# alexj94/future_urban_scene_generation

Hardware: AMD Instinct MI355X
Metric: synthesised vehicle crops/sec @256x256 (higher is better)
Workload: dtype f32 tensors; conv contraction as 3 fp16 MFMA products of scaled (hi, lo) operand splits, f32 accumulate (error vs fp64 <= 1.3x the exact-f32 MFMA kernel's: observed 0.96-1.27x over 12 operand scales x 5 layers; range-guarded; exact-f32 leg in precision_legs)

## Files before the change

future_urban_scene_generation_amd/csrc/conv_bneck.hip:

```cpp
#include "conv_kernel_h3.h"

namespace fusg {

struct BneckK {
    const float* x; const float* res; float* dst;
    long xsn, xsh, xsw, rsn, rsh, rsw, dsn, dsh, dsw;
    const float* pre_scale; const float* pre_shift;
    const _Float16* w1; const _Float16* w2; const _Float16* w3;
    const float* b1; const float* b2; const float* b3;
    const float* s1; const float* s2; const float* s3;
    const float* zeros;
    int* status;
    int B, H, W, Cin, tiles_x, tiles_y;
    int touch_w;
};

constexpr int BN_HP = 100;
constexpr int BN_SROWS = 112;
constexpr size_t bneck_lds(int planes) { return (size_t)(2 * BN_SROWS * 32 + 2 * (planes / 32) * BN_HP * 32) * sizeof(_Float16); }

template <int CT> struct WFrag { h8 f[CT][2]; };

#ifdef FUSG_BNECK_STAMPS
__device__ unsigned long long g_bneck_stamps[64 * 12];
#define FUSG_STAMP(i) do { if (threadIdx.x == 0 && blockIdx.x < 64) g_bneck_stamps[blockIdx.x * 12 + (i)] = __builtin_amdgcn_s_memtime(); } while (0)
#define FUSG_STAMP_RT(i) do { if (threadIdx.x == 0 && blockIdx.x < 64) g_bneck_stamps[blockIdx.x * 12 + (i)] = __builtin_amdgcn_s_memrealtime(); } while (0)
#else
#define FUSG_STAMP(i) do {} while (0)
#define FUSG_STAMP_RT(i) do {} while (0)
#endif

__device__ __forceinline__ f32x4 mfma16(const h8 a, const h8 b, const f32x4 c) {
    return __builtin_amdgcn_mfma_f32_16x16x32_f16(a, b, c, 0, 0, 0);
}

template <int P>
__global__ __launch_bounds__(256, 2) void hg_bneck_h3(const BneckK k) {
    constexpr int NCH = P / 32;
    constexpr int CT1 = P / 64, CT3 = P / 32;
    extern __shared__ __attribute__((aligned(16))) _Float16 smem_h[];
    _Float16* Sh = smem_h;
    _Float16* Sl = Sh + BN_SROWS * 32;
    _Float16* Th = Sl + BN_SROWS * 32;
    _Float16* Tl = Th + NCH * BN_HP * 32;
    _Float16* Uh = Th;
    _Float16* Ul = Th + NCH * 64 * 32;

    const int t = threadIdx.x, lane = t & 63, wave = t >> 6;
    const int lp = lane & 15, lg = lane >> 4;
    FUSG_STAMP_RT(8);
    FUSG_STAMP(0);
    const int tile = xcd_tile();
    const int tpi = k.tiles_x * k.tiles_y;
    const int b = tile / tpi, t2 = tile - b * tpi;
    const int ty = t2 / k.tiles_x, tx = t2 - ty * k.tiles_x;
    const int oy0 = ty * 8, ox0 = tx * 8;
    float amax = 0.f;
    const float ninf = -__builtin_inff();

    if (k.touch_w && gridDim.x <= TOUCH_MAX_WGS / 2) {
        void* dummy = (char*)smem_h + bneck_lds(P);
        const long n1 = (long)(k.Cin >> 5) * NCH * 4096, n2 = (long)9 * NCH * NCH * 4096, n3 = (long)NCH * 2 * NCH * 4096;
        for (long o = (long)t * 128; o < n1; o += 256 * 128) l2_touch((const char*)k.w1 + o, dummy);
        for (long o = (long)t * 128; o < n2; o += 256 * 128) l2_touch((const char*)k.w2 + o, dummy);
        for (long o = (long)t * 128; o < n3; o += 256 * 128) l2_touch((const char*)k.w3 + o, dummy);
    }

    const int kc = t & 7;
    const float* xp[4];
    int soff[4];
    unsigned sval = 0, sexist = 0;
#pragma unroll
    for (int j = 0; j < 4; ++j) {
        const int item = t + 256 * j, pix = item >> 3;
        xp[j] = k.zeros;
        soff[j] = 0;
        if (item < BN_SROWS * 8) {
            sexist |= 1u << j;
            soff[j] = pix * 32 + ((((kc >> 1) ^ (((pix >> 2) & 1) << 1)) << 3) | ((kc & 1) << 2));
            if (pix < BN_HP) {
                const int hy = pix / 10, hx = pix - hy * 10;
                const int iy = oy0 - 1 + hy, ix = ox0 - 1 + hx;
                if ((unsigned)iy < (unsigned)k.H && (unsigned)ix < (unsigned)k.W) {
                    sval |= 1u << j;
                    xp[j] = k.x + (long)b * k.xsn + (long)iy * k.xsh + (long)ix * k.xsw + kc * 4;
                }
            }
        }
    }
    f32x4 hreg[4], sc = {1.f, 1.f, 1.f, 1.f}, sh = {0.f, 0.f, 0.f, 0.f};
    auto issue = [&](int c) {
        sc = *(const f32x4*)(k.pre_scale + c * 32 + kc * 4);
        sh = *(const f32x4*)(k.pre_shift + c * 32 + kc * 4);
#pragma unroll
        for (int j = 0; j < 4; ++j) hreg[j] = *(const f32x4*)(((sval >> j) & 1u) ? xp[j] + c * 32 : k.zeros);
    };
    auto commit = [&]() {
#pragma unroll
        for (int j = 0; j < 4; ++j) {
            f32x4 v = hreg[j];
            const bool ok = (sval >> j) & 1u;
#pragma unroll
            for (int c = 0; c < 4; ++c) { const float y = fmaf(v[c], sc[c], sh[c]); v[c] = ok ? y : 0.f; }
            h4 hi, lo;
            split4(v, 0.f, hi, lo, amax);
            if ((sexist >> j) & 1u) { *(h4*)(Sh + soff[j]) = hi; *(h4*)(Sl + soff[j]) = lo; }
        }
    };
    auto load_w = [&](auto& F, const _Float16* w, int slab, int nt32, int gct0) {
        constexpr int CT = sizeof(F.f) / sizeof(F.f[0]);
#pragma unroll
        for (int j = 0; j < CT; ++j) {
            const int gct = gct0 + j;
            const _Float16* p = w + ((long)((slab * nt32 + (gct >> 1)) * 2 + (gct & 1)) * 2) * 512 + lane * 8;
            F.f[j][0] = *(const h8*)(p);
            F.f[j][1] = *(const h8*)(p + 512);
        }
    };

    f32x4 acc1[7][CT1];
#pragma unroll
    for (int i = 0; i < 7; ++i)
#pragma unroll
        for (int j = 0; j < CT1; ++j) acc1[i][j] = f32x4{0.f, 0.f, 0.f, 0.f};
    const int sfrag = lp * 32 + ((lg ^ (((lp >> 2) & 1) << 1)) << 3);
    auto compute1 = [&](const WFrag<CT1>& F) {
        h8 bs[CT1];
#pragma unroll
        for (int j = 0; j < CT1; ++j) bs[j] = scale_m11(F.f[j][0]);
#pragma unroll
        for (int i0 = 0; i0 < 7; i0 += 2) {
            const int n = i0 + 1 < 7 ? 2 : 1;
            h8 xh[2], xl[2];
#pragma unroll
            for (int i = 0; i < 2; ++i)
                if (i < n) { xh[i] = *(const h8*)(Sh + (i0 + i) * 512 + sfrag); xl[i] = *(const h8*)(Sl + (i0 + i) * 512 + sfrag); }
#pragma unroll
            for (int term = 0; term < 3; ++term)
#pragma unroll
                for (int i = 0; i < 2; ++i)
                    if (i < n) {
#pragma unroll
                        for (int j = 0; j < CT1; ++j)
                            acc1[i0 + i][j] = mfma16(term == 0 ? F.f[j][0] : term == 1 ? F.f[j][1] : bs[j], term == 2 ? xl[i] : xh[i], acc1[i0 + i][j]);
                    }
        }
    };

    const int nch1 = k.Cin >> 5;
    WFrag<CT1> wA, wB;
    FUSG_STAMP(1);
    issue(0);
    load_w(wA, k.w1, 0, NCH, wave * CT1);
    for (int c = 0; c < nch1; c += 2) {
        commit();
        __syncthreads();
        if (c + 1 < nch1) { issue(c + 1); load_w(wB, k.w1, c + 1, NCH, wave * CT1); }
        compute1(wA);
        __syncthreads();
        if (c + 1 >= nch1) break;
        commit();
        __syncthreads();
        if (c + 2 < nch1) { issue(c + 2); load_w(wA, k.w1, c + 2, NCH, wave * CT1); }
        compute1(wB);
        __syncthreads();
    }

    FUSG_STAMP(2);
    WFrag<CT1> w0, w1, w2;
    load_w(w0, k.w2, 0, NCH, wave * CT1);
    load_w(w1, k.w2, NCH, NCH, wave * CT1);
    const int sub = (lg & 1) << 2;
    {
#pragma unroll
        for (int j = 0; j < CT1; ++j) {
            const int gct = wave * CT1 + j;
            const int n0 = gct * 16 + lg * 4;
            const f32x4 bias = *(const f32x4*)(k.b1 + n0), wsc = *(const f32x4*)(k.s1 + n0);
            const int g = (gct & 1) * 2 + (lg >> 1);
#pragma unroll
            for (int i = 0; i < 7; ++i) {
                const int pix = i * 16 + lp;
                const int hy = pix / 10, hx = pix - hy * 10;
                const int iy = oy0 - 1 + hy, ix = ox0 - 1 + hx;
                const bool ok = pix < BN_HP && (unsigned)iy < (unsigned)k.H && (unsigned)ix < (unsigned)k.W;
                f32x4 v;
#pragma unroll
                for (int r = 0; r < 4; ++r) { const float y = fmaxf(fmaf(acc1[i][j][r], wsc[r], bias[r]), 0.f); v[r] = ok ? y : 0.f; }
                h4 hi, lo;
                split4<false>(v, ninf, hi, lo, amax);
                if (pix < BN_HP) {
                    const int o = ((gct >> 1) * BN_HP + pix) * 32 + ((g ^ ((hy & 1) << 1)) << 3) + sub;
                    *(h4*)(Th + o) = hi;
                    *(h4*)(Tl + o) = lo;
                }
            }
        }
    }
    __syncthreads();
    FUSG_STAMP(3);

    f32x4 acc2[4][CT1];
#pragma unroll
    for (int i = 0; i < 4; ++i)
#pragma unroll
        for (int j = 0; j < CT1; ++j) acc2[i][j] = f32x4{0.f, 0.f, 0.f, 0.f};
    const int prow = lp >> 3, pcol = lp & 7;
    const int tfrag = (prow * 10 + pcol) * 32;
    auto compute2 = [&](const WFrag<CT1>& F, int c, int tap) {
        const int ky = tap / 3, kx = tap - ky * 3;
        const int o = c * (BN_HP * 32) + tfrag + (ky * 10 + kx) * 32 + ((lg ^ (((prow + ky) & 1) << 1)) << 3);
        h8 xh[4], xl[4], bs[CT1];
#pragma unroll
        for (int i = 0; i < 4; ++i) { xh[i] = *(const h8*)(Th + o + i * 640); xl[i] = *(const h8*)(Tl + o + i * 640); }
#pragma unroll
        for (int j = 0; j < CT1; ++j) bs[j] = scale_m11(F.f[j][0]);
#pragma unroll
        for (int term = 0; term < 3; ++term)
#pragma unroll
            for (int i = 0; i < 4; ++i)
#pragma unroll
                for (int j = 0; j < CT1; ++j)
                    acc2[i][j] = mfma16(term == 0 ? F.f[j][0] : term == 1 ? F.f[j][1] : bs[j], term == 2 ? xl[i] : xh[i], acc2[i][j]);
    };
    for (int c = 0; c < NCH; ++c) {
#pragma unroll
        for (int tap = 0; tap < 9; tap += 3) {
            const int s2 = c * 9 + tap + 2;
            auto slab_of = [](int s) { const int cc = s / 9; return (s - cc * 9) * NCH + cc; };
            load_w(w2, k.w2, slab_of(s2), NCH, wave * CT1);
            compute2(w0, c, tap);
            if (s2 + 1 < NCH * 9) load_w(w0, k.w2, slab_of(s2 + 1), NCH, wave * CT1);
            compute2(w1, c, tap + 1);
            if (s2 + 2 < NCH * 9) load_w(w1, k.w2, slab_of(s2 + 2), NCH, wave * CT1);
            compute2(w2, c, tap + 2);
        }
    }
    FUSG_STAMP(4);
    __syncthreads();

    WFrag<CT3> v0, v1;
    load_w(v0, k.w3, 0, 2 * NCH, wave * CT3);
    {
#pragma unroll
        for (int j = 0; j < CT1; ++j) {
            const int gct = wave * CT1 + j;
            const int n0 = gct * 16 + lg * 4;
            const f32x4 bias = *(const f32x4*)(k.b2 + n0), wsc = *(const f32x4*)(k.s2 + n0);
            const int g = (gct & 1) * 2 + (lg >> 1);
#pragma unroll
            for (int i = 0; i < 4; ++i) {
                f32x4 v;
#pragma unroll
                for (int r = 0; r < 4; ++r) v[r] = fmaxf(fmaf(acc2[i][j][r], wsc[r], bias[r]), 0.f);
                h4 hi, lo;
                split4<false>(v, ninf, hi, lo, amax);
                const int o = ((gct >> 1) * 64 + i * 16 + lp) * 32 + ((g ^ (((lp >> 2) & 1) << 1)) << 3) + sub;
                *(h4*)(Uh + o) = hi;
                *(h4*)(Ul + o) = lo;
            }
        }
    }
    __syncthreads();
    FUSG_STAMP(5);

    f32x4 acc3[4][CT3];
#pragma unroll
    for (int i = 0; i < 4; ++i)
#pragma unroll
        for (int j = 0; j < CT3; ++j) acc3[i][j] = f32x4{0.f, 0.f, 0.f, 0.f};
    auto compute3 = [&](const WFrag<CT3>& F, int c) {
        h8 xh[4], xl[4];
#pragma unroll
        for (int i = 0; i < 4; ++i) { xh[i] = *(const h8*)(Uh + c * 2048 + i * 512 + sfrag); xl[i] = *(const h8*)(Ul + c * 2048 + i * 512 + sfrag); }
        h8 bs[CT3];
#pragma unroll
        for (int j = 0; j < CT3; ++j) bs[j] = scale_m11(F.f[j][0]);
#pragma unroll
        for (int term = 0; term < 3; ++term)
#pragma unroll
            for (int i = 0; i < 4; ++i)
#pragma unroll
                for (int j = 0; j < CT3; ++j)
                    acc3[i][j] = mfma16(term == 0 ? F.f[j][0] : term == 1 ? F.f[j][1] : bs[j], term == 2 ? xl[i] : xh[i], acc3[i][j]);
    };
#pragma unroll
    for (int c = 0; c < NCH; c += 2) {
        load_w(v1, k.w3, c + 1, 2 * NCH, wave * CT3);
        compute3(v0, c);
        if (c + 2 < NCH) load_w(v0, k.w3, c + 2, 2 * NCH, wave * CT3);
        compute3(v1, c + 1);
    }

    FUSG_STAMP(6);
    if (amax >= F16X3_LIMIT && k.status) *k.status = 1;

#pragma unroll
    for (int i = 0; i < 4; ++i) {
        const int oy = oy0 + 2 * i + prow, ox = ox0 + pcol;
        if (oy >= k.H || ox >= k.W) continue;
        const float* rp = k.res + (long)b * k.rsn + (long)oy * k.rsh + (long)ox * k.rsw;
        float* dp = k.dst + (long)b * k.dsn + (long)oy * k.dsh + (long)ox * k.dsw;
#pragma unroll
        for (int j = 0; j < CT3; ++j) {
            const int n0 = (wave * CT3 + j) * 16 + lg * 4;
            const f32x4 bias = *(const f32x4*)(k.b3 + n0), wsc = *(const f32x4*)(k.s3 + n0);
            const f32x4 r = *(const f32x4*)(rp + n0);
            f32x4 v;
#pragma unroll
            for (int e = 0; e < 4; ++e) v[e] = fmaf(acc3[i][j][e], wsc[e], bias[e]) + r[e];
            *(f32x4*)(dp + n0) = v;
        }
    }
    FUSG_STAMP(7);
    FUSG_STAMP_RT(9);
}


template <int CT> struct WFragF { f32x4 f[CT][2]; };

template <int P>
__global__ __launch_bounds__(256, 2) void hg_bneck_f32(const BneckK k) {
    constexpr int NCH = P / 32;
    constexpr int CT1 = P / 64, CT3 = P / 32;
    extern __shared__ __attribute__((aligned(16))) float smem_f[];
    float* S = smem_f;
    float* T = S + BN_SROWS * 32;
    float* U = T;

    const int t = threadIdx.x, lane = t & 63, wave = t >> 6;
    const int lp = lane & 15, lg = lane >> 4;
    const int tile = xcd_tile();
    const int tpi = k.tiles_x * k.tiles_y;
    const int b = tile / tpi, t2 = tile - b * tpi;
    const int ty = t2 / k.tiles_x, tx = t2 - ty * k.tiles_x;
    const int oy0 = ty * 8, ox0 = tx * 8;
    const float* w1 = (const float*)k.w1; const float* w2 = (const float*)k.w2; const float* w3 = (const float*)k.w3;

    const int kc = t & 7;
    const float* xp[4];
    int soff[4];
    unsigned sval = 0, sexist = 0;
#pragma unroll
    for (int j = 0; j < 4; ++j) {
        const int item = t + 256 * j, pix = item >> 3;
        xp[j] = k.zeros;
        soff[j] = 0;
        if (item < BN_SROWS * 8) {
            sexist |= 1u << j;
            soff[j] = pix * 32 + kc * 4;
            if (pix < BN_HP) {
                const int hy = pix / 10, hx = pix - hy * 10;
                const int iy = oy0 - 1 + hy, ix = ox0 - 1 + hx;
                if ((unsigned)iy < (unsigned)k.H && (unsigned)ix < (unsigned)k.W) {
                    sval |= 1u << j;
                    xp[j] = k.x + (long)b * k.xsn + (long)iy * k.xsh + (long)ix * k.xsw + kc * 4;
                }
            }
        }
    }
    f32x4 hreg[4], sc = {1.f, 1.f, 1.f, 1.f}, sh = {0.f, 0.f, 0.f, 0.f};
    auto issue = [&](int c) {
        sc = *(const f32x4*)(k.pre_scale + c * 32 + kc * 4);
        sh = *(const f32x4*)(k.pre_shift + c * 32 + kc * 4);
#pragma unroll
        for (int j = 0; j < 4; ++j) hreg[j] = *(const f32x4*)(((sval >> j) & 1u) ? xp[j] + c * 32 : k.zeros);
    };
    auto commit = [&]() {
#pragma unroll
        for (int j = 0; j < 4; ++j) {
            f32x4 v = hreg[j];
            const bool ok = (sval >> j) & 1u;
#pragma unroll
            for (int c = 0; c < 4; ++c) { const float y = fmaxf(fmaf(v[c], sc[c], sh[c]), 0.f); v[c] = ok ? y : 0.f; }
            if ((sexist >> j) & 1u) *(f32x4*)(S + soff[j]) = v;
        }
    };
    auto load_w = [&](auto& F, const float* w, int slab, int nt32, int gct0) {
        constexpr int CT = sizeof(F.f) / sizeof(F.f[0]);
#pragma unroll
        for (int j = 0; j < CT; ++j) {
            const int gct = gct0 + j;
            const float* p = w + ((long)((slab * nt32 + (gct >> 1)) * 2 + (gct & 1)) * 2) * 256 + lane * 4;
            F.f[j][0] = *(const f32x4*)(p);
            F.f[j][1] = *(const f32x4*)(p + 256);
        }
    };
    auto mac = [&](auto& acc_row, const auto& F, const f32x4 xa, const f32x4 xb) __attribute__((always_inline)) {
        constexpr int CT = sizeof(F.f) / sizeof(F.f[0]);
#pragma unroll
        for (int h = 0; h < 2; ++h)
#pragma unroll
            for (int e = 0; e < 4; ++e)
#pragma unroll
                for (int j = 0; j < CT; ++j)
                    acc_row[j] = __builtin_amdgcn_mfma_f32_16x16x4f32(F.f[j][h][e], h ? xb[e] : xa[e], acc_row[j], 0, 0, 0);
    };

    f32x4 acc1[7][CT1];
#pragma unroll
    for (int i = 0; i < 7; ++i)
#pragma unroll
        for (int j = 0; j < CT1; ++j) acc1[i][j] = f32x4{0.f, 0.f, 0.f, 0.f};
    const int sfrag = lp * 32 + lg * 4;
    auto compute1 = [&](const WFragF<CT1>& F) {
#pragma unroll
        for (int i = 0; i < 7; ++i) {
            const f32x4 xa = *(const f32x4*)(S + i * 512 + sfrag), xb = *(const f32x4*)(S + i * 512 + sfrag + 16);
            mac(acc1[i], F, xa, xb);
        }
    };

    const int nch1 = k.Cin >> 5;
    WFragF<CT1> wA, wB;
    issue(0);
    load_w(wA, w1, 0, NCH, wave * CT1);
    for (int c = 0; c < nch1; c += 2) {
        commit();
        __syncthreads();
        if (c + 1 < nch1) { issue(c + 1); load_w(wB, w1, c + 1, NCH, wave * CT1); }
        compute1(wA);
        __syncthreads();
        if (c + 1 >= nch1) break;
        commit();
        __syncthreads();
        if (c + 2 < nch1) { issue(c + 2); load_w(wA, w1, c + 2, NCH, wave * CT1); }
        compute1(wB);
        __syncthreads();
    }

    WFragF<CT1> w0, w1f, w2f;
    load_w(w0, w2, 0, NCH, wave * CT1);
    load_w(w1f, w2, NCH, NCH, wave * CT1);
    {
#pragma unroll
        for (int j = 0; j < CT1; ++j) {
            const int gct = wave * CT1 + j;
            const int n0 = gct * 16 + lg * 4;
            const f32x4 bias = *(const f32x4*)(k.b1 + n0);
#pragma unroll
            for (int i = 0; i < 7; ++i) {
                const int pix = i * 16 + lp;
                const int hy = pix / 10, hx = pix - hy * 10;
                const int iy = oy0 - 1 + hy, ix = ox0 - 1 + hx;
                const bool ok = pix < BN_HP && (unsigned)iy < (unsigned)k.H && (unsigned)ix < (unsigned)k.W;
                f32x4 v;
#pragma unroll
                for (int r = 0; r < 4; ++r) { const float y = fmaxf(acc1[i][j][r] + bias[r], 0.f); v[r] = ok ? y : 0.f; }
                if (pix < BN_HP) *(f32x4*)(T + ((gct >> 1) * BN_HP + pix) * 32 + (gct & 1) * 16 + lg * 4) = v;
            }
        }
    }
    __syncthreads();

    f32x4 acc2[4][CT1];
#pragma unroll
    for (int i = 0; i < 4; ++i)
#pragma unroll
        for (int j = 0; j < CT1; ++j) acc2[i][j] = f32x4{0.f, 0.f, 0.f, 0.f};
    const int prow = lp >> 3, pcol = lp & 7;
    const int tfrag = (prow * 10 + pcol) * 32 + lg * 4;
    auto compute2 = [&](const WFragF<CT1>& F, int c, int tap) {
        const int ky = tap / 3, kx = tap - ky * 3;
        const int o = c * (BN_HP * 32) + tfrag + (ky * 10 + kx) * 32;
#pragma unroll
        for (int i = 0; i < 4; ++i) {
            const f32x4 xa = *(const f32x4*)(T + o + i * 640), xb = *(const f32x4*)(T + o + i * 640 + 16);
            mac(acc2[i], F, xa, xb);
        }
    };
    for (int c = 0; c < NCH; ++c) {
#pragma unroll
        for (int tap = 0; tap < 9; tap += 3) {
            const int s2 = c * 9 + tap + 2;
            auto slab_of = [](int s) { const int cc = s / 9; return (s - cc * 9) * NCH + cc; };
            load_w(w2f, w2, slab_of(s2), NCH, wave * CT1);
            compute2(w0, c, tap);
            if (s2 + 1 < NCH * 9) load_w(w0, w2, slab_of(s2 + 1), NCH, wave * CT1);
            compute2(w1f, c, tap + 1);
            if (s2 + 2 < NCH * 9) load_w(w1f, w2, slab_of(s2 + 2), NCH, wave * CT1);
            compute2(w2f, c, tap + 2);
        }
    }
    __syncthreads();

    WFragF<CT3> v0, v1;
    load_w(v0, w3, 0, 2 * NCH, wave * CT3);
    {
#pragma unroll
        for (int j = 0; j < CT1; ++j) {
            const int gct = wave * CT1 + j;
            const int n0 = gct * 16 + lg * 4;
            const f32x4 bias = *(const f32x4*)(k.b2 + n0);
#pragma unroll
            for (int i = 0; i < 4; ++i) {
                f32x4 v;
#pragma unroll
                for (int r = 0; r < 4; ++r) v[r] = fmaxf(acc2[i][j][r] + bias[r], 0.f);
                *(f32x4*)(U + ((gct >> 1) * 64 + i * 16 + lp) * 32 + (gct & 1) * 16 + lg * 4) = v;
            }
        }
    }
    __syncthreads();

    f32x4 acc3[4][CT3];
#pragma unroll
    for (int i = 0; i < 4; ++i)
#pragma unroll
        for (int j = 0; j < CT3; ++j) acc3[i][j] = f32x4{0.f, 0.f, 0.f, 0.f};
    auto compute3 = [&](const WFragF<CT3>& F, int c) {
#pragma unroll
        for (int i = 0; i < 4; ++i) {
            const f32x4 xa = *(const f32x4*)(U + c * 2048 + i * 512 + sfrag), xb = *(const f32x4*)(U + c * 2048 + i * 512 + sfrag + 16);
            mac(acc3[i], F, xa, xb);
        }
    };
#pragma unroll
    for (int c = 0; c < NCH; c += 2) {
        load_w(v1, w3, c + 1, 2 * NCH, wave * CT3);
        compute3(v0, c);
        if (c + 2 < NCH) load_w(v0, w3, c + 2, 2 * NCH, wave * CT3);
        compute3(v1, c + 1);
    }

#pragma unroll
    for (int i = 0; i < 4; ++i) {
        const int oy = oy0 + 2 * i + prow, ox = ox0 + pcol;
        if (oy >= k.H || ox >= k.W) continue;
        const float* rp = k.res + (long)b * k.rsn + (long)oy * k.rsh + (long)ox * k.rsw;
        float* dp = k.dst + (long)b * k.dsn + (long)oy * k.dsh + (long)ox * k.dsw;
#pragma unroll
        for (int j = 0; j < CT3; ++j) {
            const int n0 = (wave * CT3 + j) * 16 + lg * 4;
            const f32x4 bias = *(const f32x4*)(k.b3 + n0);
            const f32x4 r = *(const f32x4*)(rp + n0);
            f32x4 v;
#pragma unroll
            for (int e = 0; e < 4; ++e) v[e] = (acc3[i][j][e] + bias[e]) + r[e];
            *(f32x4*)(dp + n0) = v;
        }
    }
}

}

using namespace fusg;

static int bneck_impl(const fusg_bneck_desc* d, void* stream) {
    hipStream_t s = (hipStream_t)stream;
    FUSG_CHECK(d != nullptr, "hg_bottleneck: null descriptor");
    const fusg_tensor& x = d->x;
    const int P = d->planes;
    FUSG_CHECK(P == 128 || P == 64, "hg_bottleneck: planes %d (64 and 128 are built)", d->planes);
    FUSG_CHECK(is_nhwc(x) && x.c % 32 == 0 && x.c >= 32 && x.c <= 4096, "hg_bottleneck: x must be NHWC-physical f32 with c %% 32 == 0");
    FUSG_CHECK(is_nhwc(d->res) && is_nhwc(d->dst) && same_nhw(x, d->res) && same_nhw(x, d->dst) && d->res.c == 2 * P &&
               d->dst.c == 2 * P, "hg_bottleneck: res / dst must be NHWC-physical f32 [n, 2 * planes, h, w] like x");
    FUSG_CHECK(x.data != d->dst.data && d->res.data != d->dst.data, "hg_bottleneck: dst must not alias x or res (neighbouring patches read x's halo)");
    const bool f32 = d->exact_f32 == 1;
    FUSG_CHECK(d->exact_f32 == 0 || d->exact_f32 == 1, "hg_bottleneck: exact_f32 %d", d->exact_f32);
    const void* ptrs[] = {d->pre_scale, d->pre_shift, d->w1frag, d->bias1, d->w2frag, d->bias2, d->w3frag, d->bias3};
    for (const void* p : ptrs) FUSG_CHECK(p && (((uintptr_t)p) & 15) == 0, "hg_bottleneck: a parameter array is missing or not 16-byte aligned");
    if (!f32) {
        const void* sp[] = {d->wscale1, d->wscale2, d->wscale3};
        for (const void* p : sp) FUSG_CHECK(p && (((uintptr_t)p) & 15) == 0, "hg_bottleneck: a weight-scale array is missing or not 16-byte aligned");
        FUSG_CHECK(d->status != nullptr, "hg_bottleneck: status word missing");
    }
    FUSG_CHECK(x.n * x.h * x.w * x.sw < (1L << 40) && x.n >= 1 && x.h >= 1 && x.w >= 1, "hg_bottleneck: extent");
    BneckK k;
    memset(&k, 0, sizeof(k));
    k.x = (const float*)x.data; k.res = (const float*)d->res.data; k.dst = (float*)d->dst.data;
    k.xsn = x.sn; k.xsh = x.sh; k.xsw = x.sw;
    k.rsn = d->res.sn; k.rsh = d->res.sh; k.rsw = d->res.sw;
    k.dsn = d->dst.sn; k.dsh = d->dst.sh; k.dsw = d->dst.sw;
    k.pre_scale = d->pre_scale; k.pre_shift = d->pre_shift;
    k.w1 = (const _Float16*)d->w1frag; k.w2 = (const _Float16*)d->w2frag; k.w3 = (const _Float16*)d->w3frag;
    k.b1 = d->bias1; k.b2 = d->bias2; k.b3 = d->bias3;
    k.s1 = d->wscale1; k.s2 = d->wscale2; k.s3 = d->wscale3;
    k.status = d->status;
    k.zeros = zero_line();
    if (!k.zeros) { set_error("hg_bottleneck: cannot allocate the zero line"); return FUSG_ERR_LAUNCH; }
    k.B = (int)x.n; k.H = (int)x.h; k.W = (int)x.w; k.Cin = (int)x.c;
    k.tiles_x = (k.W + 7) / 8; k.tiles_y = (k.H + 7) / 8;
    const long wgs = (long)k.B * k.tiles_x * k.tiles_y;
    FUSG_CHECK(wgs < (1L << 31), "hg_bottleneck: grid");
    const void* fn = f32 ? (P == 128 ? (const void*)hg_bneck_f32<128> : (const void*)hg_bneck_f32<64>)
                         : (P == 128 ? (const void*)hg_bneck_h3<128> : (const void*)hg_bneck_h3<64>);
    const size_t lds = bneck_lds(P) + TOUCH_LDS_BYTES;
    k.touch_w = env_switches().no_touch ? 0 : 1;
    const double M = (double)x.n * x.h * x.w;
    prof_begin(0, s, 2.0 * M * ((double)x.c * P + 9.0 * P * P + 2.0 * P * P));
    const hipError_t e = launch_kernel(fn, dim3((unsigned)wgs), lds, (int)lds, k, s);
    prof_end(0, s);
    if (e != hipSuccess) { set_error("hg_bottleneck launch: %s", hipGetErrorString(e)); return FUSG_ERR_LAUNCH; }
    note_conv_kernel(FUSG_CONV_BNECK);
    return FUSG_OK;
}
extern "C" int fusg_hg_bottleneck(const fusg_bneck_desc* d, void* stream) { return fusg::plan_dispatch(bneck_impl, stream, d); }
#ifdef FUSG_BNECK_STAMPS
extern "C" int fusg_debug_bneck_stamps(unsigned long long* out) {
    return hipMemcpyFromSymbol(out, HIP_SYMBOL(fusg::g_bneck_stamps), sizeof(unsigned long long) * 64 * 12) == hipSuccess ? 0 : 1;
}
#endif
```

Measured before the change: 1492.

## Add 8x16 patch variant of fused bottleneck kernel with 512-thread workgroups

Templates the fused bottleneck kernel on patch width and adds a 16-wide variant using 8 waves. Each group of four waves handles one 8x8 half and the halves share the staged halo and weight fragments. This cuts the halo overhead (10x18 instead of 10x10 per 64 pixels) and halves per-tile weight fetches. The cost is more LDS per workgroup and lower occupancy (one block of 512 threads per launch bound). The wide variant is chosen automatically for width divisible by 16 and large spatial sizes, with an environment override.

```diff
diff --git a/future_urban_scene_generation_amd/csrc/conv_bneck.hip b/future_urban_scene_generation_amd/csrc/conv_bneck.hip
--- a/future_urban_scene_generation_amd/csrc/conv_bneck.hip
+++ b/future_urban_scene_generation_amd/csrc/conv_bneck.hip
@@ -15,9 +15,12 @@
     int touch_w;
 };
 
-constexpr int BN_HP = 100;
-constexpr int BN_SROWS = 112;
-constexpr size_t bneck_lds(int planes) { return (size_t)(2 * BN_SROWS * 32 + 2 * (planes / 32) * BN_HP * 32) * sizeof(_Float16); }
+constexpr int bn_hp(int pw) { return 10 * (pw + 2); }
+constexpr int bn_srows(int pw) { return (bn_hp(pw) + 15) / 16 * 16; }
+constexpr size_t bneck_lds(int planes, int pw) {
+    return (size_t)(2 * bn_srows(pw) * 32 + 2 * (planes / 32) * bn_hp(pw) * 32) * sizeof(_Float16);
+}
+constexpr int BN_HP = bn_hp(8), BN_SROWS = bn_srows(8);
 
 template <int CT> struct WFrag { h8 f[CT][2]; };
 
@@ -34,52 +37,59 @@
     return __builtin_amdgcn_mfma_f32_16x16x32_f16(a, b, c, 0, 0, 0);
 }
 
-template <int P>
-__global__ __launch_bounds__(256, 2) void hg_bneck_h3(const BneckK k) {
+template <int P, int PW>
+__global__ __launch_bounds__(PW * 32, 16 / PW) void hg_bneck_h3(const BneckK k) {
     constexpr int NCH = P / 32;
     constexpr int CT1 = P / 64, CT3 = P / 32;
+    constexpr int NT = PW * 32;
+    constexpr int HW_ = PW + 2, BN_HP = bn_hp(PW), BN_SROWS = bn_srows(PW);
+    constexpr int RG1 = BN_SROWS / 16 / (PW / 8);
+    constexpr int NJ = (BN_SROWS * 8 + NT - 1) / NT;
+    constexpr int NPIX = 8 * PW;
     extern __shared__ __attribute__((aligned(16))) _Float16 smem_h[];
     _Float16* Sh = smem_h;
     _Float16* Sl = Sh + BN_SROWS * 32;
     _Float16* Th = Sl + BN_SROWS * 32;
     _Float16* Tl = Th + NCH * BN_HP * 32;
     _Float16* Uh = Th;
-    _Float16* Ul = Th + NCH * 64 * 32;
+    _Float16* Ul = Th + NCH * NPIX * 32;
 
     const int t = threadIdx.x, lane = t & 63, wave = t >> 6;
     const int lp = lane & 15, lg = lane >> 4;
+    const int cw = PW == 8 ? wave : wave & 3;
+    const int ph = PW == 8 ? 0 : wave >> 2;
     FUSG_STAMP_RT(8);
     FUSG_STAMP(0);
     const int tile = xcd_tile();
     const int tpi = k.tiles_x * k.tiles_y;
     const int b = tile / tpi, t2 = tile - b * tpi;
     const int ty = t2 / k.tiles_x, tx = t2 - ty * k.tiles_x;
-    const int oy0 = ty * 8, ox0 = tx * 8;
+    const int oy0 = ty * 8, ox0 = tx * PW;
     float amax = 0.f;
     const float ninf = -__builtin_inff();
 
     if (k.touch_w && gridDim.x <= TOUCH_MAX_WGS / 2) {
-        void* dummy = (char*)smem_h + bneck_lds(P);
+        void* dummy = (char*)smem_h + bneck_lds(P, PW);
         const long n1 = (long)(k.Cin >> 5) * NCH * 4096, n2 = (long)9 * NCH * NCH * 4096, n3 = (long)NCH * 2 * NCH * 4096;
-        for (long o = (long)t * 128; o < n1; o += 256 * 128) l2_touch((const char*)k.w1 + o, dummy);
-        for (long o = (long)t * 128; o < n2; o += 256 * 128) l2_touch((const char*)k.w2 + o, dummy);
-        for (long o = (long)t * 128; o < n3; o += 256 * 128) l2_touch((const char*)k.w3 + o, dummy);
+        for (long o = (long)t * 128; o < n1; o += NT * 128) l2_touch((const char*)k.w1 + o, dummy);
+        for (long o = (long)t * 128; o < n2; o += NT * 128) l2_touch((const char*)k.w2 + o, dummy);
+        for (long o = (long)t * 128; o < n3; o += NT * 128) l2_touch((const char*)k.w3 + o, dummy);
     }
 
     const int kc = t & 7;
-    const float* xp[4];
-    int soff[4];
+    const float* xp[NJ];
+    int soff[NJ];
     unsigned sval = 0, sexist = 0;
 #pragma unroll
-    for (int j = 0; j < 4; ++j) {
-        const int item = t + 256 * j, pix = item >> 3;
+    for (int j = 0; j < NJ; ++j) {
+        const int item = t + NT * j, pix = item >> 3;
         xp[j] = k.zeros;
         soff[j] = 0;
         if (item < BN_SROWS * 8) {
             sexist |= 1u << j;
             soff[j] = pix * 32 + ((((kc >> 1) ^ (((pix >> 2) & 1) << 1)) << 3) | ((kc & 1) << 2));
             if (pix < BN_HP) {
-                const int hy = pix / 10, hx = pix - hy * 10;
+                const int hy = pix / HW_, hx = pix - hy * HW_;
                 const int iy = oy0 - 1 + hy, ix = ox0 - 1 + hx;
                 if ((unsigned)iy < (unsigned)k.H && (unsigned)ix < (unsigned)k.W) {
                     sval |= 1u << j;
@@ -88,16 +98,16 @@
             }
         }
     }
-    f32x4 hreg[4], sc = {1.f, 1.f, 1.f, 1.f}, sh = {0.f, 0.f, 0.f, 0.f};
+    f32x4 hreg[NJ], sc = {1.f, 1.f, 1.f, 1.f}, sh = {0.f, 0.f, 0.f, 0.f};
     auto issue = [&](int c) {
         sc = *(const f32x4*)(k.pre_scale + c * 32 + kc * 4);
         sh = *(const f32x4*)(k.pre_shift + c * 32 + kc * 4);
 #pragma unroll
-        for (int j = 0; j < 4; ++j) hreg[j] = *(const f32x4*)(((sval >> j) & 1u) ? xp[j] + c * 32 : k.zeros);
+        for (int j = 0; j < NJ; ++j) hreg[j] = *(const f32x4*)(((sval >> j) & 1u) ? xp[j] + c * 32 : k.zeros);
     };
     auto commit = [&]() {
 #pragma unroll
-        for (int j = 0; j < 4; ++j) {
+        for (int j = 0; j < NJ; ++j) {
             f32x4 v = hreg[j];
             const bool ok = (sval >> j) & 1u;
 #pragma unroll
@@ -118,9 +128,9 @@
         }
     };
 
-    f32x4 acc1[7][CT1];
-#pragma unroll
-    for (int i = 0; i < 7; ++i)
+    f32x4 acc1[RG1][CT1];
+#pragma unroll
+    for (int i = 0; i < RG1; ++i)
 #pragma unroll
         for (int j = 0; j < CT1; ++j) acc1[i][j] = f32x4{0.f, 0.f, 0.f, 0.f};
     const int sfrag = lp * 32 + ((lg ^ (((lp >> 2) & 1) << 1)) << 3);
@@ -129,12 +139,12 @@
 #pragma unroll
         for (int j = 0; j < CT1; ++j) bs[j] = scale_m11(F.f[j][0]);
 #pragma unroll
-        for (int i0 = 0; i0 < 7; i0 += 2) {
-            const int n = i0 + 1 < 7 ? 2 : 1;
+        for (int i0 = 0; i0 < RG1; i0 += 2) {
+            const int n = i0 + 1 < RG1 ? 2 : 1;
             h8 xh[2], xl[2];
 #pragma unroll
             for (int i = 0; i < 2; ++i)
-                if (i < n) { xh[i] = *(const h8*)(Sh + (i0 + i) * 512 + sfrag); xl[i] = *(const h8*)(Sl + (i0 + i) * 512 + sfrag); }
+                if (i < n) { xh[i] = *(const h8*)(Sh + (ph * RG1 + i0 + i) * 512 + sfrag); xl[i] = *(const h8*)(Sl + (ph * RG1 + i0 + i) * 512 + sfrag); }
 #pragma unroll
             for (int term = 0; term < 3; ++term)
 #pragma unroll
@@ -151,37 +161,37 @@
     WFrag<CT1> wA, wB;
     FUSG_STAMP(1);
     issue(0);
-    load_w(wA, k.w1, 0, NCH, wave * CT1);
+    load_w(wA, k.w1, 0, NCH, cw * CT1);
     for (int c = 0; c < nch1; c += 2) {
         commit();
         __syncthreads();
-        if (c + 1 < nch1) { issue(c + 1); load_w(wB, k.w1, c + 1, NCH, wave * CT1); }
+        if (c + 1 < nch1) { issue(c + 1); load_w(wB, k.w1, c + 1, NCH, cw * CT1); }
         compute1(wA);
         __syncthreads();
         if (c + 1 >= nch1) break;
         commit();
         __syncthreads();
-        if (c + 2 < nch1) { issue(c + 2); load_w(wA, k.w1, c + 2, NCH, wave * CT1); }
+        if (c + 2 < nch1) { issue(c + 2); load_w(wA, k.w1, c + 2, NCH, cw * CT1); }
         compute1(wB);
         __syncthreads();
     }
 
     FUSG_STAMP(2);
     WFrag<CT1> w0, w1, w2;
-    load_w(w0, k.w2, 0, NCH, wave * CT1);
-    load_w(w1, k.w2, NCH, NCH, wave * CT1);
+    load_w(w0, k.w2, 0, NCH, cw * CT1);
+    load_w(w1, k.w2, NCH, NCH, cw * CT1);
     const int sub = (lg & 1) << 2;
     {
 #pragma unroll
         for (int j = 0; j < CT1; ++j) {
-            const int gct = wave * CT1 + j;
+            const int gct = cw * CT1 + j;
             const int n0 = gct * 16 + lg * 4;
             const f32x4 bias = *(const f32x4*)(k.b1 + n0), wsc = *(const f32x4*)(k.s1 + n0);
             const int g = (gct & 1) * 2 + (lg >> 1);
 #pragma unroll
-            for (int i = 0; i < 7; ++i) {
-                const int pix = i * 16 + lp;
-                const int hy = pix / 10, hx = pix - hy * 10;
+            for (int i = 0; i < RG1; ++i) {
+                const int pix = (ph * RG1 + i) * 16 + lp;
+                const int hy = pix / HW_, hx = pix - hy * HW_;
                 const int iy = oy0 - 1 + hy, ix = ox0 - 1 + hx;
                 const bool ok = pix < BN_HP && (unsigned)iy < (unsigned)k.H && (unsigned)ix < (unsigned)k.W;
                 f32x4 v;
@@ -206,13 +216,13 @@
 #pragma unroll
         for (int j = 0; j < CT1; ++j) acc2[i][j] = f32x4{0.f, 0.f, 0.f, 0.f};
     const int prow = lp >> 3, pcol = lp & 7;
-    const int tfrag = (prow * 10 + pcol) * 32;
+    const int tfrag = (prow * HW_ + ph * 8 + pcol) * 32;
     auto compute2 = [&](const WFrag<CT1>& F, int c, int tap) {
         const int ky = tap / 3, kx = tap - ky * 3;
-        const int o = c * (BN_HP * 32) + tfrag + (ky * 10 + kx) * 32 + ((lg ^ (((prow + ky) & 1) << 1)) << 3);
+        const int o = c * (BN_HP * 32) + tfrag + (ky * HW_ + kx) * 32 + ((lg ^ (((prow + ky) & 1) << 1)) << 3);
         h8 xh[4], xl[4], bs[CT1];
 #pragma unroll
-        for (int i = 0; i < 4; ++i) { xh[i] = *(const h8*)(Th + o + i * 640); xl[i] = *(const h8*)(Tl + o + i * 640); }
+        for (int i = 0; i < 4; ++i) { xh[i] = *(const h8*)(Th + o + i * (2 * HW_ * 32)); xl[i] = *(const h8*)(Tl + o + i * (2 * HW_ * 32)); }
 #pragma unroll
         for (int j = 0; j < CT1; ++j) bs[j] = scale_m11(F.f[j][0]);
 #pragma unroll
@@ -228,11 +238,11 @@
         for (int tap = 0; tap < 9; tap += 3) {
             const int s2 = c * 9 + tap + 2;
             auto slab_of = [](int s) { const int cc = s / 9; return (s - cc * 9) * NCH + cc; };
-            load_w(w2, k.w2, slab_of(s2), NCH, wave * CT1);
+            load_w(w2, k.w2, slab_of(s2), NCH, cw * CT1);
             compute2(w0, c, tap);
-            if (s2 + 1 < NCH * 9) load_w(w0, k.w2, slab_of(s2 + 1), NCH, wave * CT1);
+            if (s2 + 1 < NCH * 9) load_w(w0, k.w2, slab_of(s2 + 1), NCH, cw * CT1);
             compute2(w1, c, tap + 1);
-            if (s2 + 2 < NCH * 9) load_w(w1, k.w2, slab_of(s2 + 2), NCH, wave * CT1);
+            if (s2 + 2 < NCH * 9) load_w(w1, k.w2, slab_of(s2 + 2), NCH, cw * CT1);
             compute2(w2, c, tap + 2);
         }
     }
@@ -240,11 +250,11 @@
     __syncthreads();
 
     WFrag<CT3> v0, v1;
-    load_w(v0, k.w3, 0, 2 * NCH, wave * CT3);
+    load_w(v0, k.w3, 0, 2 * NCH, cw * CT3);
     {
 #pragma unroll
         for (int j = 0; j < CT1; ++j) {
-            const int gct = wave * CT1 + j;
+            const int gct = cw * CT1 + j;
             const int n0 = gct * 16 + lg * 4;
             const f32x4 bias = *(const f32x4*)(k.b2 + n0), wsc = *(const f32x4*)(k.s2 + n0);
             const int g = (gct & 1) * 2 + (lg >> 1);
@@ -255,7 +265,7 @@
                 for (int r = 0; r < 4; ++r) v[r] = fmaxf(fmaf(acc2[i][j][r], wsc[r], bias[r]), 0.f);
                 h4 hi, lo;
                 split4<false>(v, ninf, hi, lo, amax);
-                const int o = ((gct >> 1) * 64 + i * 16 + lp) * 32 + ((g ^ (((lp >> 2) & 1) << 1)) << 3) + sub;
+                const int o = ((gct >> 1) * NPIX + (ph * 4 + i) * 16 + lp) * 32 + ((g ^ (((lp >> 2) & 1) << 1)) << 3) + sub;
                 *(h4*)(Uh + o) = hi;
                 *(h4*)(Ul + o) = lo;
             }
@@ -272,7 +282,7 @@
     auto compute3 = [&](const WFrag<CT3>& F, int c) {
         h8 xh[4], xl[4];
 #pragma unroll
-        for (int i = 0; i < 4; ++i) { xh[i] = *(const h8*)(Uh + c * 2048 + i * 512 + sfrag); xl[i] = *(const h8*)(Ul + c * 2048 + i * 512 + sfrag); }
+        for (int i = 0; i < 4; ++i) { xh[i] = *(const h8*)(Uh + c * (NPIX * 32) + (ph * 4 + i) * 512 + sfrag); xl[i] = *(const h8*)(Ul + c * (NPIX * 32) + (ph * 4 + i) * 512 + sfrag); }
         h8 bs[CT3];
 #pragma unroll
         for (int j = 0; j < CT3; ++j) bs[j] = scale_m11(F.f[j][0]);
@@ -286,9 +296,9 @@
     };
 #pragma unroll
     for (int c = 0; c < NCH; c += 2) {
-        load_w(v1, k.w3, c + 1, 2 * NCH, wave * CT3);
+        load_w(v1, k.w3, c + 1, 2 * NCH, cw * CT3);
         compute3(v0, c);
-        if (c + 2 < NCH) load_w(v0, k.w3, c + 2, 2 * NCH, wave * CT3);
+        if (c + 2 < NCH) load_w(v0, k.w3, c + 2, 2 * NCH, cw * CT3);
         compute3(v1, c + 1);
     }
 
@@ -297,13 +307,13 @@
 
 #pragma unroll
     for (int i = 0; i < 4; ++i) {
-        const int oy = oy0 + 2 * i + prow, ox = ox0 + pcol;
+        const int oy = oy0 + 2 * i + prow, ox = ox0 + ph * 8 + pcol;
         if (oy >= k.H || ox >= k.W) continue;
         const float* rp = k.res + (long)b * k.rsn + (long)oy * k.rsh + (long)ox * k.rsw;
         float* dp = k.dst + (long)b * k.dsn + (long)oy * k.dsh + (long)ox * k.dsw;
 #pragma unroll
         for (int j = 0; j < CT3; ++j) {
-            const int n0 = (wave * CT3 + j) * 16 + lg * 4;
+            const int n0 = (cw * CT3 + j) * 16 + lg * 4;
             const f32x4 bias = *(const f32x4*)(k.b3 + n0), wsc = *(const f32x4*)(k.s3 + n0);
             const f32x4 r = *(const f32x4*)(rp + n0);
             f32x4 v;
@@ -546,7 +556,16 @@
 
 using namespace fusg;
 
-static int bneck_impl(const fusg_bneck_desc* d, void* stream) {
+static int bneck_patch_w(const fusg_bneck_desc* d) {
+    if (d == nullptr || d->exact_f32 != 0) return 8;
+    if (const char* e = getenv("FUSG_BNECK_PW")) {
+        const int v = atoi(e);
+        if (v == 8 || v == 16) return v;
+    }
+    return d->x.w % 16 == 0 && d->x.h * d->x.w >= 32 * 32 ? 16 : 8;
+}
+
+static int bneck_impl(const fusg_bneck_desc* d, int pw, void* stream) {
     hipStream_t s = (hipStream_t)stream;
     FUSG_CHECK(d != nullptr, "hg_bottleneck: null descriptor");
     const fusg_tensor& x = d->x;
@@ -580,22 +599,26 @@
     k.zeros = zero_line();
     if (!k.zeros) { set_error("hg_bottleneck: cannot allocate the zero line"); return FUSG_ERR_LAUNCH; }
     k.B = (int)x.n; k.H = (int)x.h; k.W = (int)x.w; k.Cin = (int)x.c;
-    k.tiles_x = (k.W + 7) / 8; k.tiles_y = (k.H + 7) / 8;
+    FUSG_CHECK((pw == 8 || pw == 16) && !(f32 && pw != 8), "hg_bottleneck: patch width %d", pw);
+    k.tiles_x = (k.W + pw - 1) / pw; k.tiles_y = (k.H + 7) / 8;
     const long wgs = (long)k.B * k.tiles_x * k.tiles_y;
     FUSG_CHECK(wgs < (1L << 31), "hg_bottleneck: grid");
     const void* fn = f32 ? (P == 128 ? (const void*)hg_bneck_f32<128> : (const void*)hg_bneck_f32<64>)
-                         : (P == 128 ? (const void*)hg_bneck_h3<128> : (const void*)hg_bneck_h3<64>);
-    const size_t lds = bneck_lds(P) + TOUCH_LDS_BYTES;
+                   : pw == 16 ? (P == 128 ? (const void*)hg_bneck_h3<128, 16> : (const void*)hg_bneck_h3<64, 16>)
+                              : (P == 128 ? (const void*)hg_bneck_h3<128, 8> : (const void*)hg_bneck_h3<64, 8>);
+    const size_t lds = bneck_lds(P, pw) + TOUCH_LDS_BYTES;
     k.touch_w = env_switches().no_touch ? 0 : 1;
     const double M = (double)x.n * x.h * x.w;
     prof_begin(0, s, 2.0 * M * ((double)x.c * P + 9.0 * P * P + 2.0 * P * P));
-    const hipError_t e = launch_kernel(fn, dim3((unsigned)wgs), lds, (int)lds, k, s);
+    hipError_t e = ensure_dyn_lds(fn, (int)lds);
+    void* args[] = {(void*)&k};
+    if (e == hipSuccess) e = hipLaunchKernel(fn, dim3((unsigned)wgs), dim3(pw * 32), args, lds, s);
     prof_end(0, s);
     if (e != hipSuccess) { set_error("hg_bottleneck launch: %s", hipGetErrorString(e)); return FUSG_ERR_LAUNCH; }
     note_conv_kernel(FUSG_CONV_BNECK);
     return FUSG_OK;
 }
-extern "C" int fusg_hg_bottleneck(const fusg_bneck_desc* d, void* stream) { return fusg::plan_dispatch(bneck_impl, stream, d); }
+extern "C" int fusg_hg_bottleneck(const fusg_bneck_desc* d, void* stream) { return fusg::plan_dispatch(bneck_impl, stream, d, bneck_patch_w(d)); }
 #ifdef FUSG_BNECK_STAMPS
 extern "C" int fusg_debug_bneck_stamps(unsigned long long* out) {
     return hipMemcpyFromSymbol(out, HIP_SYMBOL(fusg::g_bneck_stamps), sizeof(unsigned long long) * 64 * 12) == hipSuccess ? 0 : 1;
```

Measured after the change: 1444. 0.967x the previous value.
